# michelbarbeau/gr-uwspr

Hardware: AMD Instinct MI355X
Metric: 2-min WSPR frames decoded/sec (coarse+sync) (higher is better)
Workload: dtype f32

## Files before the change

gr-uwspr_amd/csrc/fft512_lane.h:

```cpp
#pragma once

#ifdef __HIPCC__
#define UWSPR_HD __host__ __device__ __forceinline__
#else
#define UWSPR_HD inline
#endif

namespace uwspr {

struct cpx { float r, i; };

UWSPR_HD int rev3(int x) { return ((x & 1) << 2) | (x & 2) | ((x >> 2) & 1); }
UWSPR_HD int rev6(int x) { return (rev3(x & 7) << 3) | rev3((x >> 3) & 7); }

UWSPR_HD int xidx(int p) {
  return p ^ ((((p >> 7) & 1) << 4) | (((p >> 6) & 1) << 3) | (((p >> 8) & 1) << 2) | (((p >> 7) & 1) << 1) |
              ((p >> 5) & 1));
}
constexpr int XCHG_LEN = 512;

UWSPR_HD void bfly(cpx &u, cpx &v, float wr, float wi) {
  float tr = wr * v.r - wi * v.i;
  float ti = wr * v.i + wi * v.r;
  float ur = u.r, ui = u.i;
  u.r = ur + tr; u.i = ui + ti;
  v.r = ur - tr; v.i = ui - ti;
}
UWSPR_HD void bfly1(cpx &u, cpx &v) {
  float tr = v.r, ti = v.i, ur = u.r, ui = u.i;
  u.r = ur + tr; u.i = ui + ti;
  v.r = ur - tr; v.i = ui - ti;
}
UWSPR_HD void bflymi(cpx &u, cpx &v) {
  float tr = v.i, ti = -v.r, ur = u.r, ui = u.i;
  u.r = ur + tr; u.i = ui + ti;
  v.r = ur - tr; v.i = ui - ti;
}

struct pass_tw { cpx s1, s2[2], s3[4]; };

UWSPR_HD pass_tw load_pass_tw(const cpx *tw, int unit, int hs) {
  pass_tw t;
  t.s1 = tw[unit * (256 / hs)];
#pragma unroll
  for (int e = 0; e < 2; e++) t.s2[e] = tw[(hs * e + unit) * (256 / (2 * hs))];
#pragma unroll
  for (int e = 0; e < 4; e++) t.s3[e] = tw[(hs * e + unit) * (256 / (4 * hs))];
  return t;
}

UWSPR_HD void pass_a(cpx y[8], cpx w64, cpx w192) {
  bfly1(y[0], y[1]); bfly1(y[2], y[3]); bfly1(y[4], y[5]); bfly1(y[6], y[7]);
  bfly1(y[0], y[2]); bflymi(y[1], y[3]); bfly1(y[4], y[6]); bflymi(y[5], y[7]);
  bfly1(y[0], y[4]);
  bfly(y[1], y[5], w64.r, w64.i);
  bflymi(y[2], y[6]);
  bfly(y[3], y[7], w192.r, w192.i);
}

UWSPR_HD void pass_bc(cpx v[8], const pass_tw &t) {
#pragma unroll
  for (int e = 0; e < 8; e += 2) bfly(v[e], v[e + 1], t.s1.r, t.s1.i);
#pragma unroll
  for (int g = 0; g < 8; g += 4) {
    bfly(v[g + 0], v[g + 2], t.s2[0].r, t.s2[0].i);
    bfly(v[g + 1], v[g + 3], t.s2[1].r, t.s2[1].i);
  }
#pragma unroll
  for (int e = 0; e < 4; e++) bfly(v[e], v[e + 4], t.s3[e].r, t.s3[e].i);
}

UWSPR_HD void bfly_sum(cpx &u, const cpx &v, float wr, float wi) {
  float tr = wr * v.r - wi * v.i;
  float ti = wr * v.i + wi * v.r;
  u.r = u.r + tr; u.i = u.i + ti;
}
UWSPR_HD void bfly_diff(const cpx &u, cpx &v, float wr, float wi) {
  float tr = wr * v.r - wi * v.i;
  float ti = wr * v.i + wi * v.r;
  v.r = u.r - tr; v.i = u.i - ti;
}
UWSPR_HD void pass_c_narrow(cpx v[8], const pass_tw &t) {
#pragma unroll
  for (int e = 0; e < 8; e += 2) bfly(v[e], v[e + 1], t.s1.r, t.s1.i);
  bfly_sum(v[0], v[2], t.s2[0].r, t.s2[0].i);
  bfly_sum(v[4], v[6], t.s2[0].r, t.s2[0].i);
  bfly_diff(v[1], v[3], t.s2[1].r, t.s2[1].i);
  bfly_diff(v[5], v[7], t.s2[1].r, t.s2[1].i);
  bfly_sum(v[0], v[4], t.s3[0].r, t.s3[0].i);
  bfly_diff(v[3], v[7], t.s3[3].r, t.s3[3].i);
}

UWSPR_HD int in_sample(int L, int r) { return L + 64 * rev3(r); }
UWSPR_HD int posA(int L, int r) { return 8 * rev6(L) + r; }
UWSPR_HD int posB(int L, int b) { return 64 * (L >> 3) + 8 * b + (L & 7); }
UWSPR_HD int posC(int L, int a) { return 64 * a + L; }
UWSPR_HD int out_col(int L, int a) { return (64 * a + L) ^ 256; }

}
```

gr-uwspr_amd/csrc/k1_spectrogram.hip:

```cpp
#include "uwspr_internal.h"
#include "fft512_lane.h"

#include <stdlib.h>

#include <type_traits>

#pragma clang fp contract(off)

namespace uwspr {

constexpr int K1_WAVES = 4;
constexpr int K1_ROWS_LARGE = 29, K1_ROWS_SMALL = 6, K1_LARGE_BATCH = 64;

__device__ __forceinline__ void k1_wave_fence() {
  __builtin_amdgcn_fence(__ATOMIC_RELEASE, "wavefront");
  __builtin_amdgcn_wave_barrier();
  __builtin_amdgcn_fence(__ATOMIC_ACQUIRE, "wavefront");
}

__device__ __forceinline__ void k1_landed(float2 &v) { asm volatile("" : "+v"(v.x), "+v"(v.y)); }
__device__ __forceinline__ constexpr int k1_slotA(int r) { return r; }
__device__ __forceinline__ constexpr int k1_slotB(int e) { return xidx(8 * e); }
__device__ __forceinline__ constexpr int k1_slotC(int a) { return xidx(64 * a); }

#ifdef UWSPR_K1_STAMPS
__device__ unsigned long long k1_stamp_buf[3 * 16384];
#define K1_STAMP(slot)                                                                      \
  if (L == 0) {                                                                             \
    const int wid = blockIdx.x * K1_WAVES + wv;                  \
    if (wid < 16384) k1_stamp_buf[3 * wid + (slot)] =                                       \
        (slot) == 2 ? ((unsigned long long)__builtin_amdgcn_s_getreg(20 | (31 << 11)) << 32) |      \
                      (unsigned)__builtin_amdgcn_s_getreg(4 | (31 << 11))                   \
                    : wall_clock64();                                                       \
  }
#else
#define K1_STAMP(slot)
#endif

template <bool NARROW>
__global__ __launch_bounds__(64 * K1_WAVES, 3) void k1_spectrogram(
    const float2 *__restrict__ frames, int B, int rpw, int fstride, int n, const float *__restrict__ window,
    const float2 *__restrict__ twiddle, float *__restrict__ ps, int band_lo, int band_w,
    int32_t *__restrict__ work_count) {
  __shared__ cpx tw_s[256];
  __shared__ cpx xch[K1_WAVES][XCHG_LEN];

  const int tid = threadIdx.x;
  const int L = tid & 63;
  const int wv = tid >> 6;
  const int gpf = (n + rpw - 1) / rpw;
  const int item = blockIdx.x * K1_WAVES + wv;
  const int b = item / gpf;
  if (blockIdx.x == 0 && tid == 0) *work_count = 0;

  K1_STAMP(0) K1_STAMP(2)
  tw_s[tid] = cpx{twiddle[tid].x, twiddle[tid].y};
  __syncthreads();

  float wreg[8];
#pragma unroll
  for (int r = 0; r < 8; r++) wreg[r] = window[in_sample(L, r)];
  const pass_tw twB = load_pass_tw(tw_s, L & 7, 8);
  const pass_tw twC = load_pass_tw(tw_s, L, 64);
  const cpx w64 = tw_s[64], w192 = tw_s[192];

  const float2 *x = frames + (size_t)b * fstride;
  cpx *lds = xch[wv];
  const int row0 = (item - b * gpf) * rpw;
  if (b >= B) { K1_STAMP(1) return; }

  float2 raw[8];
  const int laneA = xidx(posA(L, 0)), laneB = xidx(posB(L, 0)), laneC = xidx(posC(L, 0));
#pragma unroll
  for (int q = 0; q < 8; q++) raw[q] = x[row0 * 128 + L + 64 * q];
  const int rend = min(row0 + rpw, n);
  auto do_row = [&](int row, auto PH) {
    constexpr int ph = decltype(PH)::value;
    cpx y[8];
#pragma unroll
    for (int r = 0; r < 8; r++) {
      const float2 sv = raw[(rev3(r) + 2 * ph) & 7];
      y[r].r = sv.x * wreg[r];
      y[r].i = sv.y * wreg[r];
    }
    const float2 *nx = x + (row + 1 < rend ? row + 1 : row) * 128 + L;
    raw[(2 * ph) & 7] = nx[64 * 6];
    raw[(2 * ph + 1) & 7] = nx[64 * 7];
    __builtin_amdgcn_sched_barrier(0);
    pass_a(y, w64, w192);
#pragma unroll
    for (int r = 0; r < 8; r++) lds[laneA ^ k1_slotA(r)] = y[r];
    k1_wave_fence();
#pragma unroll
    for (int e = 0; e < 8; e++) y[e] = lds[laneB ^ k1_slotB(e)];
    pass_bc(y, twB);
    k1_wave_fence();
#pragma unroll
    for (int e = 0; e < 8; e++) lds[laneB ^ k1_slotB(e)] = y[e];
    k1_wave_fence();
#pragma unroll
    for (int e = 0; e < 8; e++) y[e] = lds[laneC ^ k1_slotC(e)];
    if (NARROW) pass_c_narrow(y, twC); else pass_bc(y, twC);
    k1_landed(raw[(2 * ph) & 7]); k1_landed(raw[(2 * ph + 1) & 7]);
    float *out = ps + ((size_t)b * n + row) * band_w;
#pragma unroll
    for (int e = 0; e < 8; e++) {
      if (NARROW && e != 0 && e != 7) continue;
      int col = out_col(L, e) - band_lo;
      if (col >= 0 && col < band_w) out[col] = y[e].r * y[e].r + y[e].i * y[e].i;
    }
    k1_wave_fence();
  };
  for (int row = row0; row < rend; row += 4) {
    do_row(row, std::integral_constant<int, 0>{});
    if (row + 1 < rend) do_row(row + 1, std::integral_constant<int, 1>{});
    if (row + 2 < rend) do_row(row + 2, std::integral_constant<int, 2>{});
    if (row + 3 < rend) do_row(row + 3, std::integral_constant<int, 3>{});
  }
  K1_STAMP(1)
}

#ifdef UWSPR_K1_STAMPS
extern "C" int uwspr_debug_k1_stamps(unsigned long long *out, int nwaves) {
  return (int)hipMemcpyFromSymbol(out, HIP_SYMBOL(k1_stamp_buf), sizeof(unsigned long long) * 3 * nwaves);
}
#endif

void launch_spectrogram(uwspr_ctx *c, const float *frames, int B) {
  const fdr_consts &f = c->fc;
  prof_scope ps(c, UWSPR_K_SPECTROGRAM, B);
  int rpw = B >= K1_LARGE_BATCH ? K1_ROWS_LARGE : K1_ROWS_SMALL;
  if (c->opt[UWSPR_OPT_K1_ROWS] > 0) rpw = c->opt[UWSPR_OPT_K1_ROWS];
  const int items = B * ((f.n + rpw - 1) / rpw);
  dim3 grid((items + K1_WAVES - 1) / K1_WAVES);
  const bool narrow = f.band_lo >= 192 && f.band_lo + f.band_w <= 320;
  auto go = [&](auto kern) {
    hipLaunchKernelGGL(kern, grid, dim3(64 * K1_WAVES), 0, c->stream,
                       (const float2 *)frames, B, rpw, c->fstride, f.n, c->d_window,
                       (const float2 *)c->d_twiddle, c->d_ps, f.band_lo, f.band_w, c->d_work);
  };
  if (narrow) go(k1_spectrogram<true>); else go(k1_spectrogram<false>);
}

}
```

gr-uwspr_amd/csrc/uwspr_api.hip:

```cpp
#include <errno.h>
#include <math.h>
#include <stdarg.h>
#include <stdio.h>
#include <stdlib.h>
#include <string.h>

#include <algorithm>
#include <vector>

#include "uwspr_internal.h"

namespace uwspr {
int coarse_configure(const fdr_consts &f);
size_t coarse_lds_bytes(const fdr_consts &f);
int coarse_seq_words();
size_t coarse_plan(fdr_consts &f, int pitch_opt, int tile_opt);
uint32_t coarse_seq_entry(const fdr_consts &f, int k, int off);
}

using namespace uwspr;

static int fail(uwspr_ctx *c, int status, const char *fmt, ...) {
  if (c) {
    va_list ap;
    va_start(ap, fmt);
    vsnprintf(c->err, sizeof(c->err), fmt, ap);
    va_end(ap);
  }
  return status;
}

#define HIPCHK(c, call)                                                                  \
  do {                                                                                   \
    hipError_t e_ = (call);                                                              \
    if (e_ != hipSuccess)                                                                \
      return fail((c), UWSPR_ERR_HIP, "%s failed: %s (%s:%d)", #call, hipGetErrorString(e_), \
                  __FILE__, __LINE__);                                                   \
  } while (0)

template <typename T>
static int ensure(uwspr_ctx *c, T **buf, size_t *cap, size_t need_elems) {
  if (need_elems <= *cap && *buf) return UWSPR_OK;
  if (*buf) { HIPCHK(c, hipStreamSynchronize(c->stream)); HIPCHK(c, hipFree(*buf)); *buf = nullptr; *cap = 0; }
  size_t n = std::max<size_t>(need_elems, 1);
  hipError_t e = hipMalloc((void **)buf, n * sizeof(T));
  if (e != hipSuccess) return fail(c, UWSPR_ERR_NOMEM, "hipMalloc(%zu bytes): %s", n * sizeof(T), hipGetErrorString(e));
  *cap = n;
  return UWSPR_OK;
}

prof_scope::prof_scope(uwspr_ctx *cx, int kind, int64_t units, bool ext_) : c(cx), idx(-1), ext(ext_) {
  if (!(c->prof_mask & (1 << kind))) return;
  ev_pair p;
  auto get = [&]() {
    hipEvent_t e;
    if (!c->ev_pool.empty()) { e = c->ev_pool.back(); c->ev_pool.pop_back(); }
    else (void)hipEventCreate(&e);
    return e;
  };
  p.a = get(); p.b = get(); p.kind = kind; p.units = units;
  if (!ext) (void)hipEventRecord(p.a, c->stream);
  c->prof_events.push_back(p);
  idx = (int)c->prof_events.size() - 1;
}
prof_scope::~prof_scope() {
  if (idx >= 0 && !ext) (void)hipEventRecord(c->prof_events[idx].b, c->stream);
}

static float slm_frequency_drift(double V1, double V2, int p1, int p2, float cf, float t) {
  const float cs = 1500.0f;
  const double q1 = V1 * (double)t + (double)p1;
  const double q2 = V2 * (double)t + (double)p2;
  const float sign = (float)(((q1 * V1 + q2 * V2) > 0) * 2 - 1);
  const double num = fabs(V1 * q1 + V2 * q2);
  const double den = sqrt(q1 * q1 + q2 * q2);
  if (den == 0) return 0.0f;
  return (float)((double)(-sign) * num / den * (double)cf / (double)cs);
}

static const struct { const char *name; int dflt, lo, hi; } kOptions[UWSPR_NOPT] = {
    {"sched", 1, 0, 1},
    {"stage_kernels", 1, 0, 1},
    {"reuse", 1, 0, 1},
    {"phasor_tables", 1, 0, 1},
    {"fast_search", 0, 0, 1},
    {"k4_t", 0, 0, 4},
    {"k5_lanes", -1, -1, 1},
    {"k1_rows", 0, 0, 348},
    {"k3_tile", -1, -1, 2},
    {"k3_pitch", 0, 0, 4096},
    {"sched_stamps", 0, 0, 1},
    {"sched_grid", 0, 0, 65536},
    {"dist_force_comm", 0, 0, 1},
    {"frontend", 0, 0, 1},
    {"k4_forms", 1, 0, 255},
    {"audio_rate", 12000, 8000, 192000},
    {"blank", 0, 0, 1024},
    {"blank_guard", 2, 0, 64},
    {"carrier", UWSPR_CARRIER_DEFAULT, 20, 5980},
    {"frontend_hbw", UWSPR_FRONTEND_HBW_DEFAULT, 1, 150},
};

static void refresh_options(uwspr_ctx *c) {
  c->use_stage_kernels = c->opt[UWSPR_OPT_STAGE_KERNELS] != 0;
  c->reuse_centre = c->opt[UWSPR_OPT_REUSE] != 0;
  c->use_ptab = c->opt[UWSPR_OPT_PHASOR_TABLES] != 0;
  c->fast_search = c->opt[UWSPR_OPT_FAST_SEARCH] != 0;
  c->use_fused = c->opt[UWSPR_OPT_SCHED] != 0 && !c->fast_search;
  c->sched_grid = c->opt[UWSPR_OPT_SCHED_GRID];
}

static int option_index(const char *name) {
  if (!name) return -1;
  for (int i = 0; i < UWSPR_NOPT; i++)
    if (!strcmp(name, kOptions[i].name)) return i;
  return -1;
}

extern "C" int uwspr_set_option(uwspr_ctx *c, const char *name, int value) {
  if (!c) return UWSPR_ERR_ARG;
  const int i = option_index(name);
  if (i < 0) return fail(c, UWSPR_ERR_ARG, "unknown option '%s'", name ? name : "(null)");
  if (i == UWSPR_OPT_K1_ROWS || i == UWSPR_OPT_K3_TILE || i == UWSPR_OPT_K3_PITCH)
    return fail(c, UWSPR_ERR_ARG, "option '%s' shapes the context when it is created: UWSPR_OPTIONS=%s=%d", name, name, value);
  if (value < kOptions[i].lo || value > kOptions[i].hi)
    return fail(c, UWSPR_ERR_ARG, "option '%s' = %d: allowed %d .. %d", name, value, kOptions[i].lo, kOptions[i].hi);
  if (i == UWSPR_OPT_AUDIO_RATE) {
    resample_plan pl;
    if (resample_design(value, pl))
      return fail(c, UWSPR_ERR_ARG, "option 'audio_rate' = %d: not a supported rate (12000 / gcd(rate, 12000) <= 160)", value);
  }
  if (i == UWSPR_OPT_BLANK && value != 0 && value < 4)
    return fail(c, UWSPR_ERR_ARG, "option 'blank' = %d: 0 (off) or 4 .. 1024 quarters of the median", value);
  if (i == UWSPR_OPT_CARRIER || i == UWSPR_OPT_FRONTEND_HBW || i == UWSPR_OPT_FRONTEND) {
    const int mode = i == UWSPR_OPT_FRONTEND ? value : c->opt[UWSPR_OPT_FRONTEND];
    const int fc = i == UWSPR_OPT_CARRIER ? value : c->opt[UWSPR_OPT_CARRIER];
    const int hb = i == UWSPR_OPT_FRONTEND_HBW ? value : c->opt[UWSPR_OPT_FRONTEND_HBW];
    if (!frontend_carrier_ok(mode, fc, hb))
      return fail(c, UWSPR_ERR_ARG, "option '%s' = %d: carrier %d Hz with half-bandwidth %d Hz (hb + 20 <= carrier <= 6000 - hb - 20)", name,
                  value, fc, hb);
  }
  c->opt[i] = value; c->opt_set[i] = true;
  refresh_options(c);
  return UWSPR_OK;
}

extern "C" int uwspr_get_option(uwspr_ctx *c, const char *name, int *value) {
  if (!c || !value) return UWSPR_ERR_ARG;
  const int i = option_index(name);
  if (i < 0) return fail(c, UWSPR_ERR_ARG, "unknown option '%s'", name ? name : "(null)");
  *value = c->opt[i];
  return UWSPR_OK;
}

static int options_from_environment(uwspr_ctx *c) {
  for (int i = 0; i < UWSPR_NOPT; i++) { c->opt[i] = kOptions[i].dflt; c->opt_set[i] = false; }
  const char *e = getenv("UWSPR_OPTIONS");
  if (e) {
    char buf[512];
    const size_t len = strlen(e);
    if (len >= sizeof(buf)) return fail(c, UWSPR_ERR_ARG, "UWSPR_OPTIONS: %zu characters (at most %zu)", len, sizeof(buf) - 1);
    memcpy(buf, e, len + 1);
    char *tok = buf;
    while (*tok) {
      while (*tok == ',' || *tok == ' ') tok++;
      if (!*tok) break;
      char *end = tok;
      while (*end && *end != ',' && *end != ' ') end++;
      const bool last = *end == 0;
      *end = 0;
      char *eq = strchr(tok, '=');
      if (!eq) return fail(c, UWSPR_ERR_ARG, "UWSPR_OPTIONS: '%s' is not name=value", tok);
      *eq = 0;
      const int i = option_index(tok);
      if (i < 0) return fail(c, UWSPR_ERR_ARG, "UWSPR_OPTIONS: unknown option '%s'", tok);
      char *vend = nullptr;
      errno = 0;
      const long v = strtol(eq + 1, &vend, 10);
      if (vend == eq + 1 || *vend || errno || v < kOptions[i].lo || v > kOptions[i].hi)
        return fail(c, UWSPR_ERR_ARG, "UWSPR_OPTIONS: %s='%s' is not an integer in %d .. %d", tok, eq + 1, kOptions[i].lo, kOptions[i].hi);
      if (i == UWSPR_OPT_BLANK && v != 0 && v < 4) return fail(c, UWSPR_ERR_ARG, "UWSPR_OPTIONS: blank=%ld is not 0 or 4 .. 1024", v);
      c->opt[i] = (int)v; c->opt_set[i] = true;
      if (last) break;
      tok = end + 1;
    }
  }
  refresh_options(c);
  return UWSPR_OK;
}

extern "C" int uwspr_ctx_create(const uwspr_params *p, int device, uwspr_ctx **out) {
  if (!p || !out) return UWSPR_ERR_ARG;
  *out = nullptr;
  uwspr_ctx *c = new (std::nothrow) uwspr_ctx();
  if (!c) return UWSPR_ERR_NOMEM;
  memset(c->err, 0, sizeof(c->err));
  c->p = *p;
  c->device = device;
  c->own_stream = c->stream = nullptr;
  c->d_window = c->d_twiddle = nullptr; c->d_off = nullptr; c->d_umap = nullptr; c->d_k3_tile = nullptr;
  c->d_fe_taps = nullptr; c->fe_mode = -1; c->fe_fc = 0; c->fe_hb = 0; c->fe_J = 0; c->fe_dcols = 0; c->cap_audio = 0; c->d_audio = nullptr;
  c->cap_frames_bytes = 0; c->d_frames = nullptr; c->cap_B = 0;
  c->d_ps = c->d_psavg = c->d_smraw = c->d_smspec = c->d_noise = nullptr;
  c->d_cands = nullptr; c->d_npk = nullptr; c->d_work = nullptr; c->last_B = 0; c->num_cus = 256;
  c->grid_cap = 0; c->cap_grid_bytes = 0; c->d_syncgrid = nullptr;
  c->cap_hyps = 0; c->d_hyps = nullptr; c->cap_grps = 0; c->d_grps = nullptr;
  c->cap_cent = 0; c->d_cent = nullptr; c->d_cent_frame = nullptr; c->cap_abi_hyps = 0; c->d_abi_hyps = nullptr;
  c->cap_p = 0; c->d_p = nullptr; c->cap_sync = 0; c->d_sync = nullptr;
  c->cap_sym = 0; c->d_sym = nullptr; c->cap_state = 0; c->d_state = nullptr;
  c->cap_dout = 0; c->d_dout = nullptr; c->prof_mask = 0;
  c->cur_cands = nullptr; c->cur_npk = nullptr; c->cur_dout = nullptr; c->last_per_frame = 0;
  c->cands_from_fdr = false; c->fast_now = false;
  c->cap_slab = 0; c->d_slab = nullptr;
  c->tx = nullptr;
  c->sub = nullptr;
  c->osd = nullptr;
  c->blk = nullptr;
  c->rs = nullptr;
  c->bk = nullptr;
  c->dist_comm = nullptr; c->dist_rank = 0; c->dist_world = 0;
  c->cap_tmpc = 0; c->d_tmpc = nullptr; c->cap_tmpn = 0; c->d_tmpn = nullptr;
  c->h_pin = nullptr; c->pin_busy[0] = c->pin_busy[1] = false;
  c->d_stream_frames = nullptr; c->cap_stream_frames = 0; c->ring_ev = nullptr;
  c->fstride = p->fl; c->np = p->fl < 45000 ? p->fl : 45000;
  c->cap_ptab = 0; c->d_ptab = nullptr;
  c->ntries = UWSPR_NJIG; c->cap_pwin = 0; c->d_pwin = nullptr; c->cap_need = 0; c->d_need = nullptr;
  c->last_slots = 0; c->last_sched_B = 0; c->last_sched_per_frame = 0; c->last_sched_lazy = false; c->last_sched_out = nullptr;
  c->cap_tabs = 0; c->d_tabs = nullptr; c->d_counter = nullptr; c->d_sched_stamps = nullptr; c->cap_sched_stamps = 0;
  *out = c;
  {
    const int orc = options_from_environment(c);
    if (orc) return orc;
  }

  fdr_consts &f = c->fc;
  memset(&f, 0, sizeof(f));
  const int size = 2 * p->spb;
  const int maxfreq = (int)((float)p->fs / 2.0);
  if (p->halfbandwidth > maxfreq)
    return fail(c, UWSPR_ERR_PARAM, "Half pass bandwidth (%d) must be lower than max freq range (%d)",
                p->halfbandwidth, maxfreq);
  if (p->spb != 256) return fail(c, UWSPR_ERR_UNSUPPORTED, "spb=%d: this build implements the 512-point transform (spb=256)", p->spb);
  if (p->fs <= 0 || p->fl <= 0 || p->maxdrift < 0 || p->maxfreqs < 1 || p->halfbandwidth < 1 || p->cf <= 0)
    return fail(c, UWSPR_ERR_ARG, "non-positive constructor argument");
  f.fl = p->fl; f.size = size; f.m = size / 2; f.maxfreqs = p->maxfreqs; f.maxdrift = p->maxdrift;
  f.df = (float)p->fs / (float)size;
  f.hpbm = (int)ceil((float)(int)(float)p->halfbandwidth / f.df);
  f.n = (int)(floor(((float)p->fl / (float)p->spb) * 2.0) - 3);
  f.finpb = 2 * f.hpbm;
  f.noiseidx = (int)floor(0.3 * (float)f.finpb);
  f.min_snr = (float)pow(10.0, -7.0 / 10.0);
  f.min_snr_floor = (float)(0.1 * (double)f.min_snr);
  f.threshold = (float)p->threshold;
  if (f.n < 2 * (UWSPR_NSYM - 1) + UWSPR_NK0 || (f.n - 1) * (p->spb / 2) + size > p->fl)
    return fail(c, UWSPR_ERR_UNSUPPORTED, "fl=%d too short for 162 symbols + 26 half-symbol offsets", p->fl);
  if (f.finpb > 512 || f.finpb < 3) return fail(c, UWSPR_ERR_RANGE, "pass band of %d bins", f.finpb);

  f.nlin = 2 * p->maxdrift + 1;
  f.cell_hyps = f.nlin + UWSPR_NSLM;
  f.ntot = UWSPR_NIFR * UWSPR_NK0 * f.cell_hyps;
  f.ifr_lo = f.m - f.hpbm + 1 - 2;
  const int ifr_hi = f.m + f.hpbm - 2 + 2;
  f.n_ifr = ifr_hi - f.ifr_lo + 1;
  std::vector<float> slm((size_t)UWSPR_NSLM * 111);
  for (int s = 0; s < UWSPR_NSLM; s++) {
    const double V1 = (double)((s / 5) % 5) - 2.0, V2 = (double)(s / 25) - 2.0;
    const int p2 = 50 + 200 * (s % 5);
    for (int t = 0; t < 111; t++)
      slm[(size_t)s * 111 + t] = slm_frequency_drift(V1, V2, 0, p2, (float)p->cf, (float)t);
  }
  std::vector<int8_t> off((size_t)f.n_ifr * f.cell_hyps * 164, 0);
  int omin = 1 << 30, omax = -(1 << 30);
  for (int r = 0; r < f.n_ifr; r++) {
    const int ifr = f.ifr_lo + r;
    for (int h = 0; h < f.cell_hyps; h++) {
      for (int k = 0; k < UWSPR_NSYM; k++) {
        int ifd;
        if (h < f.nlin) {
          const int drift = h - p->maxdrift;
          ifd = (int)((double)ifr + ((double)(float)k - 81.0) / 81.0 * (double)(float)drift /
                                        (2.0 * (double)f.df));
        } else {
          const int t = k * 111 / 162;
          ifd = (int)((float)ifr + slm[(size_t)(h - f.nlin) * 111 + t] / f.df);
        }
        const int o = ifd - ifr;
        if (o < -128 || o > 127) return fail(c, UWSPR_ERR_RANGE, "search reach %d bins", o);
        omin = std::min(omin, o); omax = std::max(omax, o);
        off[((size_t)r * f.cell_hyps + h) * 164 + k] = (int8_t)o;
      }
    }
  }
  f.off_min = omin; f.off_max = omax; f.nc = UWSPR_NIFR + (omax - omin);
  const int lo = std::min(f.m - f.hpbm - 3, f.ifr_lo + omin - 3);
  const int hi = std::max(f.m + f.hpbm - 1 + 3, ifr_hi + omax + 3);
  if (lo < 0 || hi > size - 1)
    return fail(c, UWSPR_ERR_RANGE,
                "halfbandwidth=%d: pass band + search reach needs columns %d..%d of 0..%d "
                "(the reference reads out of bounds here)", p->halfbandwidth, lo, hi, size - 1);
  f.band_lo = lo; f.band_w = hi - lo + 1;
  f.cand_slots = std::min(p->maxfreqs, std::max(1, (f.finpb - 1) / 2));

  int ndev = 0;
  if (hipGetDeviceCount(&ndev) != hipSuccess || ndev <= 0)
    return fail(c, UWSPR_ERR_NODEVICE, "no HIP device visible; this library has no CPU fallback");
  if (device < 0 || device >= ndev) return fail(c, UWSPR_ERR_ARG, "device %d of %d", device, ndev);
  HIPCHK(c, hipSetDevice(device));
  hipDeviceProp_t prop;
  HIPCHK(c, hipGetDeviceProperties(&prop, device));
  snprintf(c->device_name, sizeof(c->device_name), "%s", prop.gcnArchName);
  c->num_cus = prop.multiProcessorCount > 0 ? prop.multiProcessorCount : 256;
  if (strncmp(prop.gcnArchName, "gfx950", 6) != 0)
    return fail(c, UWSPR_ERR_NODEVICE, "device %d is %s; kernels are built for gfx950 only", device,
                prop.gcnArchName);
  HIPCHK(c, hipStreamCreateWithFlags(&c->own_stream, hipStreamNonBlocking));
  c->stream = c->own_stream;

  std::vector<float> w(size), tw(size);
  for (int i = 0; i < size; i++) w[i] = (float)sin((M_PI / (size - 1)) * i);
  for (int k = 0; k < size / 2; k++) {
    const double ang = 2.0 * M_PI * (double)k / 512.0;
    tw[2 * k] = (float)cos(ang);
    tw[2 * k + 1] = (float)(-sin(ang));
  }
  tw[0] = 1.0f; tw[1] = 0.0f; tw[256] = 0.0f; tw[257] = -1.0f;
  std::vector<std::vector<int>> uniq_of(f.n_ifr);
  std::vector<uint16_t> umap((size_t)f.n_ifr * f.cell_hyps);
  f.umax = 0;
  for (int r = 0; r < f.n_ifr; r++) {
    for (int h = 0; h < f.cell_hyps; h++) {
      const int8_t *sh = &off[((size_t)r * f.cell_hyps + h) * 164];
      int u = -1;
      for (size_t q = 0; q < uniq_of[r].size(); q++)
        if (memcmp(sh, &off[((size_t)r * f.cell_hyps + uniq_of[r][q]) * 164], UWSPR_NSYM) == 0) { u = (int)q; break; }
      if (u < 0) { u = (int)uniq_of[r].size(); uniq_of[r].push_back(h); }
      umap[(size_t)r * f.cell_hyps + h] = (uint16_t)u;
    }
    f.umax = std::max(f.umax, (int)uniq_of[r].size());
  }
  const size_t k3_scratch = coarse_plan(f, c->opt[UWSPR_OPT_K3_PITCH], c->opt[UWSPR_OPT_K3_TILE]);
  const int sw = coarse_seq_words();
  std::vector<uint32_t> offw((size_t)f.n_ifr * f.umax * sw, 0u);
  for (int r = 0; r < f.n_ifr; r++)
    for (int u = 0; u < f.umax; u++) {
      const int h = u < (int)uniq_of[r].size() ? uniq_of[r][u] : uniq_of[r][0];
      for (int k = 0; k < UWSPR_NSYM; k++) {
        const uint32_t e = coarse_seq_entry(f, k, off[((size_t)r * f.cell_hyps + h) * 164 + k]);
        if (e > 0xffffu) return fail(c, UWSPR_ERR_UNSUPPORTED, "coarse tile of %d centre columns", f.nc);
        offw[((size_t)r * f.umax + u) * sw + k / 2] |= e << (16 * (k & 1));
      }
    }
  if (coarse_lds_bytes(f) > 160 * 1024)
    return fail(c, UWSPR_ERR_UNSUPPORTED, "coarse search needs %zu B of LDS (> 160 KiB): reduce maxdrift/cf",
                coarse_lds_bytes(f));
  if (k3_scratch) HIPCHK(c, hipMalloc((void **)&c->d_k3_tile, k3_scratch * sizeof(float) * (size_t)c->num_cus));
  HIPCHK(c, hipMalloc((void **)&c->d_umap, umap.size() * sizeof(uint16_t)));
  HIPCHK(c, hipMemcpy(c->d_umap, umap.data(), umap.size() * sizeof(uint16_t), hipMemcpyHostToDevice));
  HIPCHK(c, hipMalloc((void **)&c->d_window, size * sizeof(float)));
  HIPCHK(c, hipMalloc((void **)&c->d_twiddle, size * sizeof(float)));
  HIPCHK(c, hipMalloc((void **)&c->d_off, offw.size() * sizeof(uint32_t)));
  HIPCHK(c, hipMemcpy(c->d_window, w.data(), size * sizeof(float), hipMemcpyHostToDevice));
  HIPCHK(c, hipMemcpy(c->d_twiddle, tw.data(), size * sizeof(float), hipMemcpyHostToDevice));
  HIPCHK(c, hipMemcpy(c->d_off, offw.data(), offw.size() * sizeof(uint32_t), hipMemcpyHostToDevice));
  if (coarse_configure(f) != 0) return fail(c, UWSPR_ERR_HIP, "cannot reserve %zu B of LDS for the coarse search", coarse_lds_bytes(f));
  return UWSPR_OK;
}

extern "C" void uwspr_ctx_destroy(uwspr_ctx *c) {
  if (!c) return;
  (void)uwspr_dist_finalize(c);
  if (c->own_stream) { (void)hipStreamSynchronize(c->own_stream); }
  tx_release(c);
  sub_release(c);
  osd_release(c);
  blk_release(c);
  rs_release(c);
  bk_release(c);
  void *bufs[] = {c->d_window, c->d_twiddle, c->d_k3_tile, c->d_off, c->d_umap, c->d_fe_taps, c->d_dbg_taps, c->d_audio, c->d_frames, c->d_ps, c->d_psavg, c->d_smraw,
                  c->d_smspec, c->d_noise, c->d_cands, c->d_npk, c->d_work, c->d_syncgrid, c->d_hyps, c->d_grps, c->d_cent,
                  c->d_abi_hyps, c->d_p, c->d_sync, c->d_sym, c->d_state, c->d_dout, c->d_slab, c->d_tabs, c->d_counter, c->d_sched_stamps, c->d_pwin, c->d_ptab, c->d_need, c->d_stream_frames, c->d_tmpc, c->d_tmpn};
  for (void *b : bufs) if (b) (void)hipFree(b);
  c->ring.close();
  if (c->ring_ev) (void)hipEventDestroy(c->ring_ev);
  if (c->h_pin) { (void)hipHostFree(c->h_pin); (void)hipEventDestroy(c->pin_ev[0]); (void)hipEventDestroy(c->pin_ev[1]); }
  for (auto &e : c->prof_events) { (void)hipEventDestroy(e.a); (void)hipEventDestroy(e.b); }
  for (auto &e : c->ev_pool) (void)hipEventDestroy(e);
  if (c->own_stream) (void)hipStreamDestroy(c->own_stream);
  delete c;
}

extern "C" const char *uwspr_last_error(const uwspr_ctx *c) { return c ? c->err : "null context"; }

extern "C" const char *uwspr_status_string(int s) {
  switch (s) {
    case UWSPR_OK: return "ok";
    case UWSPR_ERR_PARAM: return "half pass bandwidth above fs/2";
    case UWSPR_ERR_RANGE: return "pass band plus search reach outside the spectrum";
    case UWSPR_ERR_UNSUPPORTED: return "unsupported geometry";
    case UWSPR_ERR_HIP: return "HIP runtime error";
    case UWSPR_ERR_NOMEM: return "out of memory";
    case UWSPR_ERR_ARG: return "bad argument";
    case UWSPR_ERR_NODEVICE: return "no gfx950 device (no CPU fallback)";
    default: return "unknown status";
// ... 1040 lines not shown
```

gr-uwspr_amd/csrc/uwspr_internal.h:

```cpp
#pragma once

#include <hip/hip_runtime.h>
#include <hip/hip_ext.h>
#include <stdint.h>
#include <vector>

#include "../../include/uwspr_hip.h"
#include "stream_ring.h"

enum {
  UWSPR_OPT_SCHED = 0,
  UWSPR_OPT_STAGE_KERNELS,
  UWSPR_OPT_REUSE,
  UWSPR_OPT_PHASOR_TABLES,
  UWSPR_OPT_FAST_SEARCH,
  UWSPR_OPT_K4_T,
  UWSPR_OPT_K5_LANES,
  UWSPR_OPT_K1_ROWS,
  UWSPR_OPT_K3_TILE,
  UWSPR_OPT_K3_PITCH,
  UWSPR_OPT_SCHED_STAMPS,
  UWSPR_OPT_SCHED_GRID,
  UWSPR_OPT_DIST_FORCE_COMM,
  UWSPR_OPT_FRONTEND,
  UWSPR_OPT_K4_FORMS,
  UWSPR_OPT_AUDIO_RATE,
  UWSPR_OPT_BLANK,
  UWSPR_OPT_BLANK_GUARD,
  UWSPR_OPT_CARRIER,
  UWSPR_OPT_FRONTEND_HBW,
  UWSPR_NOPT
};

enum {
  UWSPR_FORM_FLAT_T1 = 0,
  UWSPR_FORM_FLAT_T2,
  UWSPR_FORM_FLAT_T4,
  UWSPR_FORM_FLAT_FAST,
  UWSPR_FORM_FOLD_WAVE,
  UWSPR_FORM_FOLD_LANES,
  UWSPR_FORM_GRID_NL1,
  UWSPR_FORM_GRID_NL2,
  UWSPR_FORM_GRID_NL4,
  UWSPR_FORM_GRID_NL5,
  UWSPR_FORM_GRID_NL6,
  UWSPR_FORM_GRID_NL8,
  UWSPR_FORM_GRID_WPW1,
  UWSPR_FORM_GRID_WPW2,
  UWSPR_FORM_GRID_WPW4,
  UWSPR_FORM_GRID_FALLBACK,
  UWSPR_FORM_FOLD_WAVE_SOFT,
  UWSPR_FORM_FOLD_LANES_SOFT,
  UWSPR_FORM_FOLD_WAVE_PWIN,
  UWSPR_FORM_FOLD_LANES_PWIN,
  UWSPR_NFORMS
};

namespace uwspr {

#define UWSPR_PR3_WORDS                                                        \
  { 0x07a47103u, 0x58b340a4u, 0x56349558u, 0xe2cdc904u, 0x63580ca0u, 0x00000000u }
__host__ __device__ constexpr uint32_t pr3_word(int w) {
  constexpr uint32_t t[6] = UWSPR_PR3_WORDS;
  return t[w];
}
__host__ __device__ constexpr int pr3_bit(int k) { return (pr3_word(k >> 5) >> (k & 31)) & 1; }

__device__ __forceinline__ float ieee_sqrtf(float x) { return __builtin_sqrtf(x); }
__device__ __forceinline__ float ieee_divf(float x, float y) { return x / y; }

__device__ __forceinline__ unsigned xcd_swizzle(unsigned bid, unsigned nwg) {
#ifdef UWSPR_NO_XCD_SWIZZLE
  return bid;
#else
  const unsigned q = nwg >> 3, r = nwg & 7u, x = bid & 7u;
  return (x < r ? x * (q + 1) : r * (q + 1) + (x - r) * q) + (bid >> 3);
#endif
}

#ifndef UWSPR_SMALL_PRIO
#define UWSPR_SMALL_PRIO 3
#endif
#define UWSPR_SET_PRIO(level) do { if ((level) > 0) __builtin_amdgcn_s_setprio(level); } while (0)

struct dev_hyp {
  int32_t frame;
  int32_t lag;
  float f0;
  float drift;
  float slmc;
  int32_t m_type;
};

struct dev_grp {
  int32_t frame;
  int32_t m_type;
  float f0, drift, slmc;
  int32_t nvalid;
  int32_t hyp_base;
  int32_t lag[8];
  uint32_t hmap;
};
static_assert(sizeof(dev_grp) == 64, "dev_grp is one 64-byte record");

struct cand_state {
  int32_t frame;
  int32_t m_type;
  float slmc;
  float f1, drift1, sync1;
  int32_t shift1;
  int32_t worth;
  float driftp, driftm;
  float csync;
  int32_t cknown;
  float tabA_f, tabB_f;
  int32_t tabA_ok, tabB_ok;
};
constexpr int kPtabPerSlot = 10;
constexpr int kPtabSetB = 5;
constexpr int kPtabFloat2 = 4 * 256;

struct fdr_consts {
  int fl, n, size, m, hpbm, finpb, noiseidx, maxfreqs, maxdrift;
  int band_lo, band_w;
  int cell_hyps, nlin, ntot;
  int off_min, off_max, nc;
  int tp;
  int k3_mode;
  int ifr_lo, n_ifr;
  int umax;
  int cand_slots;
  float df, min_snr, min_snr_floor, threshold;
};

struct ev_pair { hipEvent_t a, b; int kind; int64_t units; };
struct tx_state;
void tx_release(uwspr_ctx *c);
struct sub_state;
void sub_release(uwspr_ctx *c);
struct osd_state;
void osd_release(uwspr_ctx *c);
struct blk_state;
void blk_release(uwspr_ctx *c);
struct rs_state;
void rs_release(uwspr_ctx *c);
struct bk_state;
void bk_release(uwspr_ctx *c);

}

struct uwspr_ctx {
  uwspr_params p;
  uwspr::fdr_consts fc;
  int device;
  int num_cus;
  char device_name[64];
  hipStream_t own_stream, stream;
  char err[512];

  float *d_window;
  float *d_twiddle;
  float *d_k3_tile;
  uint32_t *d_off;
  uint16_t *d_umap;
  float *d_fe_taps;
  int fe_mode, fe_J, fe_dcols;
  int fe_fc, fe_hb;
  std::vector<int> dbg_car;
  int dbg_mode = -1, dbg_hb = 0, dbg_J = 0, dbg_dcols = 0;
  float *d_dbg_taps = nullptr;
  size_t cap_audio; float *d_audio;

  size_t cap_frames_bytes; float *d_frames;
  int cap_B;
  float *d_ps;
  float *d_psavg;
  float *d_smraw;
  float *d_smspec;
  float *d_noise;
  uwspr_candidate *d_cands;
  int32_t *d_npk;
  int32_t *d_work;
  int last_B;
  int grid_cap; size_t cap_grid_bytes; float *d_syncgrid;

  size_t cap_hyps; uwspr::dev_hyp *d_hyps;
  size_t cap_grps; uwspr::dev_grp *d_grps;
  size_t cap_cent; uwspr_candidate *d_cent; int32_t *d_cent_frame;
  size_t cap_abi_hyps; uwspr_hyp *d_abi_hyps;
  size_t cap_p; float4 *d_p;
  size_t cap_sync; float *d_sync;
  size_t cap_sym; uint8_t *d_sym;
  size_t cap_state; uwspr::cand_state *d_state;
  size_t cap_dout; uwspr_demod_out *d_dout;
  uwspr_candidate *cur_cands; int32_t *cur_npk; uwspr_demod_out *cur_dout;
  int last_per_frame;
  int opt[UWSPR_NOPT];
  bool opt_set[UWSPR_NOPT];
  long long launch_forms[UWSPR_NFORMS] = {};
  bool use_fused;
  bool use_stage_kernels;
  bool reuse_centre;
  bool use_ptab;
  bool fast_search, fast_now;
  bool cands_from_fdr;
  uint8_t *next_slab = nullptr; int next_slab_K = 0; bool next_slab_done = false;
  int sched_per_frame = 1;
  int sched_grid;
  size_t cap_tabs; float *d_tabs;
  int *d_counter;
  size_t cap_tmpc; uwspr_candidate *d_tmpc; size_t cap_tmpn; int32_t *d_tmpn;
  void *h_pin; hipEvent_t pin_ev[2]; bool pin_busy[2];
  uwspr::stream_ring ring; float *d_stream_frames; size_t cap_stream_frames;
  hipEvent_t ring_ev;
  int fstride, np;
  int ntries;
  size_t cap_ptab; float2 *d_ptab;
  size_t cap_pwin; float *d_pwin;
  size_t cap_need; uint8_t *d_need;
  int last_slots, last_sched_B, last_sched_per_frame;
  bool last_sched_lazy; uwspr_demod_out *last_sched_out;
  unsigned long long *d_sched_stamps; size_t cap_sched_stamps;
  size_t cap_slab; uint8_t *d_slab;
  void *dist_comm; int dist_rank, dist_world;
  uwspr::tx_state *tx;
  uwspr::sub_state *sub;
  uwspr::osd_state *osd;
  uwspr::blk_state *blk;
  uwspr::rs_state *rs;
  uwspr::bk_state *bk;

  int prof_mask;
  std::vector<uwspr::ev_pair> prof_events;
  std::vector<hipEvent_t> ev_pool;
};

namespace uwspr {

int api_frames_on_device(uwspr_ctx *c, const float *frames, int B, int where, const float **dev);
int subtract_check(uwspr_ctx *c, const uwspr_sub_item *items, int nitems, int nframes);
int subtract_run(uwspr_ctx *c, const float *src, size_t stride, int nslots, const int *slot_frame, const uwspr_sub_item *items,
                 int nitems, int refine, float *dst);

int osd_run(uwspr_ctx *c, const uint8_t *base, const unsigned long long *off, int n, int order, uwspr_osd_result *res,
            uwspr_osd_result **res_out);

int blockdemod_check(uwspr_ctx *c, const uwspr_block_item *items, int nitems, int nframes);
int blockdemod_run(uwspr_ctx *c, const float *src, size_t stride, const uwspr_block_item *items, int nitems, uint8_t *out,
                   uint8_t **out_dev);

int frontend_design(int mode, int stage, std::vector<double> &out, int *delay);
int frontend_tap_image(int mode, std::vector<float> &img, int *J, int *dcols);
int frontend_design_at(int mode, int fc, int hb, int stage, std::vector<double> &out, int *delay);
std::vector<float> lowpass_hamming(double fs, double cutoff, double tw);
int frontend_prepare();
double gr_izero(double x);
int rs_batch(uwspr_ctx *c, const void *audio, long long nin, int nch, int s16, int rate, int where, float *out, long long nout);
int rs_debug_launch(uwspr_ctx *c, const void *audio_dev, int s16, long long nin, long long in0, int nch, int rate, float *out_dev,
                    long long nout, long long j_first);
long long resample_launch_count(int s16);
int bk_batch(uwspr_ctx *c, const void *audio, long long nin, int nch, int s16, int where, int blank, int guard, float *out,
             float *med, int *nzero);
int bk_debug_launch(uwspr_ctx *c, const void *audio_dev, int s16, long long nin, long long in0, int nch, float *lev_dev,
                    long long nlev, long long blk0, long long level_first, long long level_n, int blank, int guard, float *out_dev,
                    long long nout, long long y_first, int *nz_dev);
long long blank_launch_count(int which);
int ring_blank_stats(stream_ring &r, long long *samples, long long *zeroed, int cap);
void launch_frontend(uwspr_ctx *c, const float *audio, int B, int nin, float2 *out, int nout);
void launch_spectrogram(uwspr_ctx *c, const float *frames, int B);
void launch_spectrum(uwspr_ctx *c, int B);
void launch_coarse(uwspr_ctx *c, int B);
void launch_prep_hyps(uwspr_ctx *c, const uwspr_hyp *abi, dev_hyp *out, int H);
void launch_tonecorr(uwspr_ctx *c, const float *frames, int B, const dev_hyp *hyps, int H,
                     float4 *p, const dev_grp *taken = nullptr, int hyps_per_grp = 1, bool skip_pairs = false);
void launch_tonecorr_dpair(uwspr_ctx *c, const float *frames, int B, const dev_hyp *hyps, int nslots, float4 *p);
void launch_tonecorr_lag0(uwspr_ctx *c, const float *frames, int B, const dev_grp *grps, int nslots,
                          int64_t nhyps, float4 *p);
void launch_tonecorr_fstage(uwspr_ctx *c, const float *frames, int B, const dev_hyp *hyps, int nslots,
                            int64_t nhyps, float4 *p);
void launch_tonecorr_ring(uwspr_ctx *c, const float *frames, int B, const dev_grp *grps, int G,
                          int NL, int step, int64_t nhyps, float4 *p, int groups_per_slot = 1);
void launch_tonecorr_jig(uwspr_ctx *c, const float *frames, int B, const dev_grp *grps, int G, int64_t nhyps, float4 *p,
                         int groups_per_slot);
bool launch_tonecorr_grid(uwspr_ctx *c, const float *frames, int B, const uwspr_candidate *centres,
                          int nf, const float *df, int ndrift, const float *ddrift, int nlag,
                          const int *dlag_host, const int *dlag_dev, dev_hyp *hyps, float4 *p);
void launch_fold(uwspr_ctx *c, const dev_hyp *hyps, const float4 *p, int H, float *sync,
                 uint8_t *symbols, const float4 *pwin = nullptr, int per_slot = 1);
void launch_keep_try0(uwspr_ctx *c, int nslots, int njig);
void launch_sched_init(uwspr_ctx *c, const uwspr_candidate *cands, const int32_t *npk,
                       int cand_stride, int B, int per_frame);
void launch_fold_step(uwspr_ctx *c, int stage, int ncand, int njig = UWSPR_NJIG);
void launch_pack_slabs(uwspr_ctx *c, const uwspr_candidate *cands, const int32_t *npk,
                       const uwspr_demod_out *dout, int per_frame, int K, uint8_t *slab, int B);
void launch_sched_finish(uwspr_ctx *c, int ncand, int njig = UWSPR_NJIG);
void launch_sched_fused(uwspr_ctx *c, const float *frames, int B, const uwspr_candidate *cands,
                        const int32_t *npk, int cand_stride, int per_frame, uwspr_demod_out *out,
                        int njig, const uint8_t *resume = nullptr);
constexpr int kSchedTabFloats = 2 * 5 * 4 * 512;

struct prof_scope {
  uwspr_ctx *c; int idx; bool ext;
  prof_scope(uwspr_ctx *c, int kind, int64_t units, bool ext = false);
  ~prof_scope();
};

template <typename K, typename... A>
inline void launch_timed(uwspr_ctx *c, prof_scope &ps, K kernel, dim3 grid, dim3 block, size_t shmem,
                         A... args) {
  if (ps.idx >= 0 && ps.ext)
    hipExtLaunchKernelGGL(kernel, grid, block, (uint32_t)shmem, c->stream, c->prof_events[ps.idx].a,
                          c->prof_events[ps.idx].b, 0, args...);
  else
    hipLaunchKernelGGL(kernel, grid, block, shmem, c->stream, args...);
}

}
```

Measured before the change: 728,600.

## Add band-pruned FFT final pass and optional register transpose in spectrogram kernel

```diff
diff --git a/gr-uwspr_amd/csrc/fft512_lane.h b/gr-uwspr_amd/csrc/fft512_lane.h
--- a/gr-uwspr_amd/csrc/fft512_lane.h
+++ b/gr-uwspr_amd/csrc/fft512_lane.h
@@ -91,6 +91,47 @@
   bfly_diff(v[3], v[7], t.s3[3].r, t.s3[3].i);
 }
 
+struct band_tw { cpx s1, s2, s3; };
+UWSPR_HD cpx cneg(cpx w) { return cpx{-w.r, -w.i}; }
+UWSPR_HD band_tw load_band_tw(const cpx *tw, int L) {
+  band_tw t;
+  if (L < 32) { t.s1 = tw[4 * L]; t.s2 = tw[2 * L]; t.s3 = tw[L]; }
+  else { t.s1 = cneg(tw[4 * L]); t.s2 = cneg(tw[2 * (64 + L)]); t.s3 = cneg(tw[192 + L]); }
+  return t;
+}
+UWSPR_HD cpx pass_c_band(cpx v[8], const band_tw &t) {
+#pragma unroll
+  for (int e = 0; e < 8; e += 2) bfly_sum(v[e], v[e + 1], t.s1.r, t.s1.i);
+  bfly_sum(v[0], v[2], t.s2.r, t.s2.i);
+  bfly_sum(v[4], v[6], t.s2.r, t.s2.i);
+  bfly_sum(v[0], v[4], t.s3.r, t.s3.i);
+  return v[0];
+}
+UWSPR_HD int band_bin(int L) { return L < 32 ? L : 448 + L; }
+UWSPR_HD int band_col(int L) { return ((L < 32 ? L : L - 64) & 511) ^ 256; }
+
+UWSPR_HD bool band_skips_b34(int band_lo, int band_w) { return band_lo >= 232 && band_lo + band_w <= 280; }
+UWSPR_HD void pass_b_band(cpx v[8], const pass_tw &t) {
+#pragma unroll
+  for (int e = 0; e < 8; e += 2) bfly(v[e], v[e + 1], t.s1.r, t.s1.i);
+#pragma unroll
+  for (int g = 0; g < 8; g += 4) {
+    bfly(v[g + 0], v[g + 2], t.s2[0].r, t.s2[0].i);
+    bfly(v[g + 1], v[g + 3], t.s2[1].r, t.s2[1].i);
+  }
+  bfly_sum(v[0], v[4], t.s3[0].r, t.s3[0].i);
+  bfly(v[1], v[5], t.s3[1].r, t.s3[1].i);
+  bfly(v[2], v[6], t.s3[2].r, t.s3[2].i);
+  bfly_diff(v[3], v[7], t.s3[3].r, t.s3[3].i);
+}
+
+UWSPR_HD void xpose_src(int s, int L, int e, int &srcL, int &srce) {
+  const int lb = 1 << (5 - s), sb = 1 << (2 - s);
+  const bool moves = (((L & lb) != 0) != ((e & sb) != 0));
+  srcL = moves ? L ^ lb : L;
+  srce = moves ? e ^ sb : e;
+}
+
 UWSPR_HD int in_sample(int L, int r) { return L + 64 * rev3(r); }
 UWSPR_HD int posA(int L, int r) { return 8 * rev6(L) + r; }
 UWSPR_HD int posB(int L, int b) { return 64 * (L >> 3) + 8 * b + (L & 7); }
diff --git a/gr-uwspr_amd/csrc/k1_spectrogram.hip b/gr-uwspr_amd/csrc/k1_spectrogram.hip
--- a/gr-uwspr_amd/csrc/k1_spectrogram.hip
+++ b/gr-uwspr_amd/csrc/k1_spectrogram.hip
@@ -37,7 +37,34 @@
 #define K1_STAMP(slot)
 #endif
 
-template <bool NARROW>
+__device__ __forceinline__ void k1_swap32(float &a, float &b) {
+  const auto r = __builtin_amdgcn_permlane32_swap(__float_as_uint(a), __float_as_uint(b), false, false);
+  a = __uint_as_float(r[0]); b = __uint_as_float(r[1]);
+}
+__device__ __forceinline__ void k1_swap16(float &a, float &b) {
+  const auto r = __builtin_amdgcn_permlane16_swap(__float_as_uint(a), __float_as_uint(b), false, false);
+  a = __uint_as_float(r[0]); b = __uint_as_float(r[1]);
+}
+__device__ __forceinline__ void k1_swap8(float &a, float &b) {
+  constexpr int ROW_ROR8 = 0x128;
+  const int ia = __float_as_int(a), ib = __float_as_int(b);
+  a = __int_as_float(__builtin_amdgcn_update_dpp(ia, ib, ROW_ROR8, 0xF, 0xC, false));
+  b = __int_as_float(__builtin_amdgcn_update_dpp(ib, ia, ROW_ROR8, 0xF, 0x3, false));
+}
+__device__ __forceinline__ void k1_xpose(cpx y[8]) {
+#pragma unroll
+  for (int e = 0; e < 8; e++)
+    if (!(e & 4)) { k1_swap32(y[e].r, y[e + 4].r); k1_swap32(y[e].i, y[e + 4].i); }
+#pragma unroll
+  for (int e = 0; e < 8; e++)
+    if (!(e & 2)) { k1_swap16(y[e].r, y[e + 2].r); k1_swap16(y[e].i, y[e + 2].i); }
+#pragma unroll
+  for (int e = 0; e < 8; e++)
+    if (!(e & 1)) { k1_swap8(y[e].r, y[e + 1].r); k1_swap8(y[e].i, y[e + 1].i); }
+}
+
+enum { K1_FULL = 0, K1_NARROW, K1_BAND };
+template <int FORM, bool XREG = false, bool B34 = false>
 __global__ __launch_bounds__(64 * K1_WAVES, 3) void k1_spectrogram(
     const float2 *__restrict__ frames, int B, int rpw, int fstride, int n, const float *__restrict__ window,
     const float2 *__restrict__ twiddle, float *__restrict__ ps, int band_lo, int band_w,
@@ -61,7 +88,10 @@
 #pragma unroll
   for (int r = 0; r < 8; r++) wreg[r] = window[in_sample(L, r)];
   const pass_tw twB = load_pass_tw(tw_s, L & 7, 8);
-  const pass_tw twC = load_pass_tw(tw_s, L, 64);
+  pass_tw twC;
+  band_tw twCb;
+  if constexpr (FORM == K1_BAND) twCb = load_band_tw(tw_s, L); else twC = load_pass_tw(tw_s, L, 64);
+  const int bcol = band_col(L) - band_lo;
   const cpx w64 = tw_s[64], w192 = tw_s[192];
 
   const float2 *x = frames + (size_t)b * fstride;
@@ -93,23 +123,37 @@
     k1_wave_fence();
 #pragma unroll
     for (int e = 0; e < 8; e++) y[e] = lds[laneB ^ k1_slotB(e)];
-    pass_bc(y, twB);
-    k1_wave_fence();
+    if constexpr (XREG) k1_wave_fence();
+    if constexpr (B34) pass_b_band(y, twB); else pass_bc(y, twB);
+    if constexpr (XREG) {
+      k1_xpose(y);
+    } else {
+      k1_wave_fence();
 #pragma unroll
-    for (int e = 0; e < 8; e++) lds[laneB ^ k1_slotB(e)] = y[e];
-    k1_wave_fence();
+      for (int e = 0; e < 8; e++) {
+        if (B34 && (e == 3 || e == 4)) continue;
+        lds[laneB ^ k1_slotB(e)] = y[e];
+      }
+      k1_wave_fence();
 #pragma unroll
-    for (int e = 0; e < 8; e++) y[e] = lds[laneC ^ k1_slotC(e)];
-    if (NARROW) pass_c_narrow(y, twC); else pass_bc(y, twC);
-    k1_landed(raw[(2 * ph) & 7]); k1_landed(raw[(2 * ph + 1) & 7]);
+      for (int e = 0; e < 8; e++) y[e] = lds[laneC ^ k1_slotC(e)];
+    }
     float *out = ps + ((size_t)b * n + row) * band_w;
+    if constexpr (FORM == K1_BAND) {
+      const cpx z = pass_c_band(y, twCb);
+      k1_landed(raw[(2 * ph) & 7]); k1_landed(raw[(2 * ph + 1) & 7]);
+      if (bcol >= 0 && bcol < band_w) out[bcol] = z.r * z.r + z.i * z.i;
+    } else {
+      if (FORM == K1_NARROW) pass_c_narrow(y, twC); else pass_bc(y, twC);
+      k1_landed(raw[(2 * ph) & 7]); k1_landed(raw[(2 * ph + 1) & 7]);
 #pragma unroll
-    for (int e = 0; e < 8; e++) {
-      if (NARROW && e != 0 && e != 7) continue;
-      int col = out_col(L, e) - band_lo;
-      if (col >= 0 && col < band_w) out[col] = y[e].r * y[e].r + y[e].i * y[e].i;
+      for (int e = 0; e < 8; e++) {
+        if (FORM == K1_NARROW && e != 0 && e != 7) continue;
+        int col = out_col(L, e) - band_lo;
+        if (col >= 0 && col < band_w) out[col] = y[e].r * y[e].r + y[e].i * y[e].i;
+      }
     }
-    k1_wave_fence();
+    if constexpr (!XREG) k1_wave_fence();
   };
   for (int row = row0; row < rend; row += 4) {
     do_row(row, std::integral_constant<int, 0>{});
@@ -134,12 +178,18 @@
   const int items = B * ((f.n + rpw - 1) / rpw);
   dim3 grid((items + K1_WAVES - 1) / K1_WAVES);
   const bool narrow = f.band_lo >= 192 && f.band_lo + f.band_w <= 320;
+  const int form = c->opt[UWSPR_OPT_K1_FORM];
+  const bool band = form > 0 && f.band_lo >= 224 && f.band_lo + f.band_w <= 288;
+  const bool b34 = band_skips_b34(f.band_lo, f.band_w);
   auto go = [&](auto kern) {
     hipLaunchKernelGGL(kern, grid, dim3(64 * K1_WAVES), 0, c->stream,
                        (const float2 *)frames, B, rpw, c->fstride, f.n, c->d_window,
                        (const float2 *)c->d_twiddle, c->d_ps, f.band_lo, f.band_w, c->d_work);
   };
-  if (narrow) go(k1_spectrogram<true>); else go(k1_spectrogram<false>);
+  if (band && form == 2) { if (b34) go(k1_spectrogram<K1_BAND, true, true>); else go(k1_spectrogram<K1_BAND, true, false>); }
+  else if (band) { if (b34) go(k1_spectrogram<K1_BAND, false, true>); else go(k1_spectrogram<K1_BAND, false, false>); }
+  else if (narrow) go(k1_spectrogram<K1_NARROW>);
+  else go(k1_spectrogram<K1_FULL>);
 }
 
 }
diff --git a/gr-uwspr_amd/csrc/uwspr_api.hip b/gr-uwspr_amd/csrc/uwspr_api.hip
--- a/gr-uwspr_amd/csrc/uwspr_api.hip
+++ b/gr-uwspr_amd/csrc/uwspr_api.hip
@@ -99,6 +99,7 @@
     {"blank_guard", 2, 0, 64},
     {"carrier", UWSPR_CARRIER_DEFAULT, 20, 5980},
     {"frontend_hbw", UWSPR_FRONTEND_HBW_DEFAULT, 1, 150},
+    {"k1_form", 1, 0, 2},
 };
 
 static void refresh_options(uwspr_ctx *c) {
diff --git a/gr-uwspr_amd/csrc/uwspr_internal.h b/gr-uwspr_amd/csrc/uwspr_internal.h
--- a/gr-uwspr_amd/csrc/uwspr_internal.h
+++ b/gr-uwspr_amd/csrc/uwspr_internal.h
@@ -29,6 +29,7 @@
   UWSPR_OPT_BLANK_GUARD,
   UWSPR_OPT_CARRIER,
   UWSPR_OPT_FRONTEND_HBW,
+  UWSPR_OPT_K1_FORM,
   UWSPR_NOPT
 };
 
```

Result: faster. 736,800 (median of 6 runs) (+1.1%).
